# skygazer42/realtime-video-analytics-32streams

Measured on AMD Instinct MI355X. Metric: aggregate detected FPS across streams + p99 per-frame latency, 32x1080p30, higher is better.
Workload: dtype f16

## Files before the change

include/rva.h:

```cpp
#ifndef RVA_H
#define RVA_H

#include <stdint.h>

#ifdef __cplusplus
extern "C" {
#endif

#define RVA_ABI_VERSION 1

enum rva_status {
    RVA_OK = 0,
    RVA_ERR_ARG = 1,
    RVA_ERR_HIP = 2,
    RVA_ERR_CAPACITY = 3,
    RVA_ERR_UNAVAILABLE = 4
};

enum rva_dtype { RVA_F16 = 0, RVA_F32 = 1, RVA_F64 = 2  };

typedef struct rva_ctx rva_ctx;
typedef struct rva_tracker rva_tracker;
typedef void *rva_stream_t;

// ... 113 lines not shown
int rva_tracker_set_next_id(rva_tracker *trk, int64_t next_id, rva_stream_t stream);

int rva_conv_cout_pad(int Cout);
int rva_conv_num_variants(void);
const char *rva_conv_variant_name(int variant);
int rva_conv2d_nhwc_f16(rva_ctx *ctx, const void *in, int ldi, const void *weights, const float *bias,
                        void *out, int ldo, const void *residual, int ldr, int batch, int H, int W, int Cin,
                        int Cout, int ksize, int stride, int act, rva_stream_t stream);
int rva_conv2d_nhwc_f16_v(rva_ctx *ctx, const void *in, int ldi, const void *weights, const float *bias,
                          void *out, int ldo, const void *residual, int ldr, int batch, int H, int W, int Cin,
                          int Cout, int ksize, int stride, int act, int variant, rva_stream_t stream);
int rva_conv2d_nhwc_f16_rows(rva_ctx *ctx, const void *in, int ldi, const void *weights, const float *bias,
                             void *out, int ldo, const void *residual, int ldr, int batch, int H, int W, int Cin,
                             int Cout, int ksize, int stride, int act, int variant, int y0, int y1, rva_stream_t stream);
int rva_conv_rows_through(int k, int stride, int H_in, int lo, int hi, int32_t *out_lo, int32_t *out_hi);
int rva_conv1x1_upcat_f16(rva_ctx *ctx, const void *low, int ld_low, int c_low, const void *skip, int ld_skip,
                          int c_skip, const void *weights, const float *bias, void *out, int ldo, int batch,
                          int H, int W, int Cout, int act, int variant, rva_stream_t stream);
int rva_conv1x1_head_f16(rva_ctx *ctx, const void *in, int ldi, const void *weights, const float *bias, int batch,
                         int H, int W, int Cin, int Cout, int mode, void *out, int nc, int anchors_total,
                         int anchor_offset, float stride_px, int variant, rva_stream_t stream);
int rva_conv1x1_head_box32_f16(rva_ctx *ctx, const void *in, int ldi, const void *weights, const float *bias, int batch,
                               int H, int W, int Cin, void *out, float *boxes32, int nc, int anchors_total, int anchor_offset,
                               float stride_px, int variant, rva_stream_t stream);
int rva_stem_conv_f16(rva_ctx *ctx, const void *in_planar, const void *weights, const float *bias,
                      void *out, int ldo, int batch, int H, int W, int Cout, rva_stream_t stream);

int rva_c2f_pair32_f16(rva_ctx *ctx, const void *in, int ldi, const void *w1, const float *b1, const void *w2, const float *b2, void *out,
                       int ldo, int batch, int H, int W, rva_stream_t stream);

// ... 255 lines not shown
```

realtime_video_analytics_32streams_amd/_native.py:

```python
from __future__ import annotations

import ctypes as C
import os
import shutil
import subprocess
from pathlib import Path
from typing import Optional

PKG = Path(__file__).resolve().parent
ROOT = PKG.parent
CSRC = PKG / "csrc"
LIB_PATH = Path(os.environ["RVA_LIB_PATH"]) if os.environ.get("RVA_LIB_PATH") else PKG / "librva.so"
SOURCES = ["rva_ctx.hip", "rva_preprocess.hip", "rva_postprocess.hip", "rva_tracker.hip", "rva_conv.hip", "rva_conv_f32.hip", "rva_plan.hip", "rva_clip.hip",
           "rva_clip3d.hip", "rva_clip3d_f16.hip", "rva_clip_f16.hip", "rva_resnet.hip", "rva_resnet_f16.hip", "rva_gates.hip", "rva_decode.hip", "rva_preview.hip", "rva_jpeg.hip"]
HIPCC_FLAGS = ["--offload-arch=gfx950", "-O3", "-fPIC", "-shared", "-std=c++17", "-ffp-contract=off",
               "-Wall", "-Wno-unused-function"]

RVA_OK, RVA_ERR_ARG, RVA_ERR_HIP, RVA_ERR_CAPACITY, RVA_ERR_UNAVAILABLE = range(5)
RVA_F16, RVA_F32, RVA_F64 = 0, 1, 2
NORM_IMAGENET_F32, NORM_VIDEO_F32, NORM_IMAGENET_F64 = 0, 1, 2
LAYOUT_NCHW, LAYOUT_CNHW = 0, 1
RVA_MAX_BATCH = 64
RVA_CODEC_H264, RVA_CODEC_HEVC = 0, 1

# ... 50 lines not shown
    _fields_ = [("y", C.c_void_p), ("uv", C.c_void_p), ("out_bgr", C.c_void_p)] + [
        (n, C.c_int32) for n in ("pitch", "src_w", "src_h", "ratio", "dst_w", "dst_h", "rect_first", "n_rects", "glyph_first", "n_glyphs")]


RVA_PLAN_NO_STEM2 = 1
RVA_PLAN_NO_CIN_PAD = 2
RVA_PLAN_NO_PAIR32 = 4
RVA_PLAN_F32 = 8
RVA_PLAN_BOX_F32 = 16


def _stale() -> bool:
    if not LIB_PATH.exists():
        return True
    t = LIB_PATH.stat().st_mtime
    deps = [CSRC / s for s in SOURCES] + [CSRC / "rva_internal.h", CSRC / "rva_plan_topo.h", CSRC / "rva_mfma_f32.h", CSRC / "rva_mfma_f16.h", ROOT / "include" / "rva.h"]
    return any(d.exists() and d.stat().st_mtime > t for d in deps)


def build(force: bool = False, verbose: bool = False) -> Path:
    if not force and not _stale():
        return LIB_PATH
    hipcc = shutil.which("hipcc") or "/opt/rocm/bin/hipcc"
    if not Path(hipcc).exists():
        if LIB_PATH.exists():
            return LIB_PATH
        raise RuntimeError("hipcc not found and librva.so is not built")
    cmd = [hipcc, *HIPCC_FLAGS, f"-I{ROOT / 'include'}", "-o", str(LIB_PATH), *[str(CSRC / s) for s in SOURCES], "-ldl"]
    if verbose:
        print(" ".join(cmd))
    subprocess.check_call(cmd, cwd=str(CSRC))
# ... 73 lines not shown
        "rva_decoder_release": (C.c_int, [_P, C.c_int]),
        "rva_motion_nv12_batch": (C.c_int, [_P, pp, pp, i32p, pp, pp, C.c_int, C.c_int, C.c_int, _P, _P]),
        "rva_motion_nv12_masked_batch": (C.c_int, [_P, pp, pp, i32p, pp, pp, pp, C.c_int, C.c_int, C.c_int, _P, _P]),
        "rva_motion_bgr_batch": (C.c_int, [_P, pp, i32p, pp, pp, C.c_int, C.c_int, C.c_int, _P, _P]),
        "rva_preprocess_nv12_masked_batch": (C.c_int, [_P, pp, pp, i32p, pp, C.c_int, C.c_int, C.c_int, _P, C.c_int, C.c_int,
                                                       C.c_int, C.POINTER(Letterbox), _P]),
        "rva_resize_nv12_to_bgr_batch": (C.c_int, [_P, pp, pp, i32p, pp, C.c_int, C.c_int, C.c_int, _P, C.c_int, C.c_int, _P]),
        "rva_tracker_set_box_scale": (C.c_int, [_P, f64p]),
        "rva_conv_cout_pad": (C.c_int, [C.c_int]),
        "rva_conv_num_variants": (C.c_int, []),
        "rva_conv_variant_name": (C.c_char_p, [C.c_int]),
        "rva_conv2d_nhwc_f16": (C.c_int, [_P, _P, C.c_int, _P, _P, _P, C.c_int, _P, C.c_int] + [C.c_int] * 8 + [_P]),
        "rva_conv2d_nhwc_f16_v": (C.c_int, [_P, _P, C.c_int, _P, _P, _P, C.c_int, _P, C.c_int] + [C.c_int] * 9 + [_P]),
        "rva_conv2d_nhwc_f16_rows": (C.c_int, [_P, _P, C.c_int, _P, _P, _P, C.c_int, _P, C.c_int] + [C.c_int] * 11 + [_P]),
        "rva_conv_rows_through": (C.c_int, [C.c_int] * 5 + [i32p, i32p]),
        "rva_stem2_f16_rows": (C.c_int, [_P, _P, _P, _P, _P, _P, _P, C.c_int, C.c_int, C.c_int, C.c_int, C.c_int, C.c_int, _P]),
        "rva_stem_conv_f16": (C.c_int, [_P, _P, _P, _P, _P, C.c_int, C.c_int, C.c_int, C.c_int, C.c_int, _P]),
        "rva_stem2_f16": (C.c_int, [_P, _P, _P, _P, _P, _P, _P, C.c_int, C.c_int, C.c_int, C.c_int, _P]),
        "rva_c2f_pair32_f16": (C.c_int, [_P, _P, C.c_int, _P, _P, _P, _P, _P, C.c_int, C.c_int, C.c_int, C.c_int, _P]),
        "rva_conv1x1_head_f16": (C.c_int, [_P, _P, C.c_int, _P, _P, C.c_int, C.c_int, C.c_int, C.c_int, C.c_int, C.c_int, _P, C.c_int,
                                           C.c_int, C.c_int, C.c_float, C.c_int, _P]),
        "rva_conv1x1_head_box32_f16": (C.c_int, [_P, _P, C.c_int, _P, _P, C.c_int, C.c_int, C.c_int, C.c_int, _P, _P, C.c_int,
                                                 C.c_int, C.c_int, C.c_float, C.c_int, _P]),
        "rva_yolo_head_box32_f16": (C.c_int, [_P, _P, C.c_int, _P, C.c_int, _P, _P, C.c_int, C.c_int, C.c_int, C.c_int, C.c_int,
                                              C.c_int, C.c_float, _P]),
        "rva_yolo_head3_box32_f16": (C.c_int, [_P, pp, i32p, pp, i32p, _P, _P, C.c_int, i32p, i32p, C.c_int, C.c_int,
                                               C.POINTER(C.c_float), _P]),
        "rva_conv1x1_upcat_f16": (C.c_int, [_P, _P, C.c_int, C.c_int, _P, C.c_int, C.c_int, _P, _P, _P, C.c_int, C.c_int, C.c_int,
                                            C.c_int, C.c_int, C.c_int, C.c_int, _P]),
        "rva_yolo_head3_f16": (C.c_int, [_P, pp, i32p, pp, i32p, _P, C.c_int, i32p, i32p, C.c_int, C.c_int, C.POINTER(C.c_float), _P]),
# ... 88 lines not shown
    "rva_tracker_set_gates", "rva_tracker_snapshot_status", "rva_tracker_new_counts",
    "rva_tracker_assign_ids", "rva_tracker_read", "rva_tracker_read_all", "rva_tracker_snapshot_async",
    "rva_tracker_snapshot_fetch", "rva_tracker_state",
    "rva_tracker_set_next_id", "rva_preview_nv12", "rva_decode_available", "rva_decoder_create", "rva_decoder_destroy", "rva_decoder_feed",
    "rva_decoder_next_frame", "rva_decoder_release", "rva_motion_nv12_batch", "rva_motion_nv12_masked_batch", "rva_motion_bgr_batch",
    "rva_preprocess_nv12_masked_batch", "rva_resize_nv12_to_bgr_batch", "rva_tracker_set_box_scale", "rva_conv_cout_pad", "rva_conv_num_variants", "rva_conv_variant_name", "rva_conv2d_nhwc_f16", "rva_conv2d_nhwc_f16_v", "rva_stem_conv_f16", "rva_stem2_f16", "rva_c2f_pair32_f16",
    "rva_conv1x1_head_f16", "rva_conv1x1_upcat_f16", "rva_sppf_pool3_nhwc_f16", "rva_maxpool5_nhwc_f16", "rva_upsample2x_nhwc_f16", "rva_yolo_head_f16", "rva_yolo_head3_f16",
    "rva_conv_f32_num_variants", "rva_conv2d_nhwc_f32_v", "rva_stem_conv_f32", "rva_maxpool5_nhwc_f32", "rva_upsample2x_nhwc_f32",
    "rva_yolo_head_f32",
    "rva_postprocess_boxes_batch", "rva_conv1x1_head_box32_f16", "rva_yolo_head_box32_f16", "rva_yolo_head3_box32_f16",
    "rva_yolov8_plan_output_layout",
    "rva_yolov8_plan_create", "rva_yolov8_plan_destroy", "rva_yolov8_plan_info", "rva_yolov8_plan_run", "rva_yolov8_plan_run_lanes",
    "rva_yolov8_plan_run_range", "rva_yolov8_plan_tunable_desc", "rva_yolov8_plan_launch_tunable", "rva_yolov8_plan_set_variant",
    "rva_yolov8_plan_get_variant", "rva_yolov8_plan_set_static_rows", "rva_yolov8_plan_step_rows", "rva_yolov8_plan_run_n",
    "rva_yolov8_plan_run_lanes_n", "rva_yolov8_plan_run_range_n", "rva_yolov8_plan_primed_images", "rva_conv2d_nhwc_f16_rows",
    "rva_stem2_f16_rows", "rva_conv_rows_through", "rva_cnnlstm_plan_create", "rva_cnnlstm_plan_destroy", "rva_cnnlstm_plan_info", "rva_cnnlstm_plan_run",
    "rva_cnnlstm_plan_run_post", "rva_cnnlstm_plan_stage", "rva_cnnlstm_f16_plan_create", "rva_cnnlstm_f16_plan_destroy", "rva_cnnlstm_f16_plan_info",
    "rva_cnnlstm_f16_plan_run", "rva_cnnlstm_f16_plan_run_post", "rva_cnnlstm_f16_plan_stage", "rva_cnn3d_plan_create", "rva_cnn3d_plan_destroy", "rva_cnn3d_plan_info", "rva_cnn3d_plan_run",
    "rva_cnn3d_plan_run_post", "rva_cnn3d_plan_stage", "rva_cnn3d_f16_plan_create", "rva_cnn3d_f16_plan_destroy", "rva_cnn3d_f16_plan_info",
    "rva_cnn3d_f16_plan_run", "rva_cnn3d_f16_plan_run_post", "rva_cnn3d_f16_plan_stage", "rva_resnet_plan_create", "rva_resnet_plan_destroy", "rva_resnet_plan_info",
    "rva_resnet_plan_run", "rva_resnet_plan_run_post", "rva_resnet_plan_stage", "rva_resnet_f16_plan_create", "rva_resnet_f16_plan_destroy",
    "rva_resnet_f16_plan_info", "rva_resnet_f16_plan_run", "rva_resnet_f16_plan_run_post", "rva_resnet_f16_plan_stage", "rva_jpeg_max_bytes", "rva_jpeg_encode_bgr", "rva_jpeg_status",
    "rva_jpeg_batch_create", "rva_jpeg_batch_destroy", "rva_jpeg_batch_encode", "rva_preview_nv12_batch",
]


class Context:

    def __init__(self, device: int = 0):
        L = lib()
        h = _P()
# ... 42 lines not shown
```

realtime_video_analytics_32streams_amd/csrc/rva_conv.hip:

```cpp
#include <hip/hip_fp16.h>

#include <cstdlib>

#include "rva_internal.h"

namespace {

typedef _Float16 h8 __attribute__((ext_vector_type(8)));
typedef float f4 __attribute__((ext_vector_type(4)));
typedef unsigned int u4 __attribute__((ext_vector_type(4)));

struct ConvArgs {
    const __half *in; int ldi;
    const __half *w;
    const float *bias;
    __half *out; int ldo;
    union {
        const __half *res;
        float *hbox;
    };
    int ldr;
    int CoutPad;
    __half *hout; int hmode, hnc, hA, ha0, hW, hHW; float hstride;
    const __half *in2; int ldi2, c_split;
// ... 1083 lines not shown
{
    static_assert(WGM * WGN == 8, "eight waves");
    static_assert(NSLOT == 2 || NSLOT == 3, "ring depth");
    constexpr int TM = BM / WGM, TN = BN / WGN, FM = TM / 16, FN = TN / 16;
    constexpr int APIECES = (BM + 2 + 15) / 16;
    constexpr int WPIECES = 3 * BN / 16;
    constexpr int PIECES = APIECES + WPIECES;
    constexpr int SLOTH = PIECES * 512;
    constexpr int NP = (PIECES + 7) / 8;
    extern __shared__ __attribute__((aligned(16))) unsigned char smem[];
    __half *ring = (__half *)smem;

    const int tid = threadIdx.x, lane = tid & 63;
    const int wv = __builtin_amdgcn_readfirstlane(tid >> 6);
    const int wm = wv % WGM, wn = wv / WGM;
    const int n_tile = (blockIdx.x >> 3) % a.n_tiles, m_tile = ((blockIdx.x >> 3) / a.n_tiles) * 8 + (blockIdx.x & 7);
    if (m_tile >= a.m_tiles) return;
    const int P0 = m_tile * BM, n0 = n_tile * BN;
    const int HW = a.H * a.W;
    const int cpt = a.Cin >> 5;
    const int nsteps = 3 * cpt;
    const int wrow = 9 * a.Cin;

    const int lrow = lane >> 2, lp = lane & 3;
    const int my_pieces = (PIECES - wv + 7) / 8;
    unsigned poff0[NP], poff1[NP], poff2[NP];
#pragma unroll
    for (int k = 0; k < NP; ++k) {
        const int idx = wv + 8 * k;
        if (idx < APIECES) {
            const int r = idx * 16 + lrow;
            const unsigned c = (unsigned)(((lp - 2 * (r >> 2)) & 3) * 16);
// ... 213 lines not shown
    int H, W, Cin, Cout, CoutPad, act, n_tiles, M, m_tiles, apieces, map_off;
};

template <int BM, int BN, int WGM, int WGN, bool NOSEL = false, bool PADO = false>
__global__ void __launch_bounds__(512) __attribute__((amdgpu_waves_per_eu(BN <= 64 && BM <= 320 ? 4 : 2))) k_conv3_run(RunArgs a)
{
    static_assert(WGM * WGN == 8, "eight waves");
    constexpr int TM = BM / WGM, TN = BN / WGN, FM = TM / 16, FN = TN / 16;
    constexpr int WPIECES = 3 * BN / 16;
    constexpr int NPW = (WPIECES + 7) / 8;
    constexpr int MAXA = 5;
    extern __shared__ __attribute__((aligned(16))) unsigned char smem[];
    const int tid = threadIdx.x, lane = tid & 63;
    const int wv = __builtin_amdgcn_readfirstlane(tid >> 6);
    const int wm = wv % WGM, wn = wv / WGM;
    const int n_tile = (blockIdx.x >> 3) % a.n_tiles, m_tile = ((blockIdx.x >> 3) / a.n_tiles) * 8 + (blockIdx.x & 7);
    if (m_tile >= a.m_tiles) return;
    const int P0 = m_tile * BM, n0 = n_tile * BN;
    const int HW = a.H * a.W;
    const int cpt = a.Cin >> 5;
    const int nsteps = 3 * cpt;
    const int wrow = 9 * a.Cin;
    const int apieces = a.apieces;
    __half *act0 = (__half *)smem;
    __half *wt0 = act0 + (size_t)2 * apieces * 512;
    const unsigned lds_act = lds_addr(act0), lds_w = lds_addr(wt0);

    const int lrow = lane >> 2, lp = lane & 3;
    unsigned aoff[MAXA], woff[NPW];
    const int Wp = PADO ? a.W + 1 : a.W, HWp = (a.H + 1) * Wp;
    const float inv_wp = 1.0f / (float)Wp, inv_hwp = 1.0f / (float)HWp;
    unsigned long long amask[PADO ? MAXA : 1];
// ... 211 lines not shown
    return hipGetLastError();
}

template <int BM, int BN, int WGM, int WGN>
__global__ void __launch_bounds__(512) __attribute__((amdgpu_waves_per_eu(BM <= 128 && BN <= 64 ? 4 : 2))) k_conv3_s2run(RunArgs a)
{
    static_assert(WGM * WGN == 8, "eight waves");
    constexpr int TM = BM / WGM, TN = BN / WGN, FM = TM / 16, FN = TN / 16;
    constexpr int WPIECES = 3 * BN / 16, NPW = (WPIECES + 7) / 8;
    constexpr int BMO = (BM + 1 + 15) / 16 * 16;
    constexpr int AP = (BMO + BM) / 16, MAXA = (AP + 7) / 8;
    extern __shared__ __attribute__((aligned(16))) unsigned char smem[];
    const int tid = threadIdx.x, lane = tid & 63;
    const int wv = __builtin_amdgcn_readfirstlane(tid >> 6);
    const int wm = wv % WGM, wn = wv / WGM;
    const int n_tile = (blockIdx.x >> 3) % a.n_tiles, m_tile = ((blockIdx.x >> 3) / a.n_tiles) * 8 + (blockIdx.x & 7);
    if (m_tile >= a.m_tiles) return;
    const int P0 = m_tile * BM, n0 = n_tile * BN;
    const int Ho = a.H >> 1, Wo = a.W >> 1, Wp = Wo + 1, HWp = Ho * Wp;
    const int cpt = a.Cin >> 5, nsteps = 3 * cpt, wrow = 9 * a.Cin;
    __half *act0 = (__half *)smem;
    __half *wt0 = act0 + (size_t)3 * AP * 512;
    const unsigned lds_act = lds_addr(act0), lds_w = lds_addr(wt0);
    const int lrow = lane >> 2, lp = lane & 3;
    const float inv_wp = 1.0f / (float)Wp, inv_hwp = 1.0f / (float)HWp;
    const int batch = a.M / (Ho * Wo);
    unsigned aoff[MAXA], woff[NPW];
    unsigned long long am1[MAXA], am0[MAXA];
#pragma unroll
    for (int k = 0; k < MAXA; ++k) {
        const int r = (wv + 8 * k) * 16 + lrow;
        const bool odd = r < BMO;
// ... 157 lines not shown
}

template <int BM, int BN, int WGM, int WGN>
__global__ void __launch_bounds__(512) __attribute__((amdgpu_waves_per_eu(2))) k_conv3_chunk(RunArgs a)
{
    static_assert(WGM * WGN == 8, "eight waves");
    constexpr int TM = BM / WGM, TN = BN / WGN, FM = TM / 16, FN = TN / 16;
    static_assert(TM % 16 == 0 && TN % 16 == 0, "whole fragments per wave");
    constexpr int WPIECES = 9 * BN / 16;
    constexpr int NPW = (WPIECES + 7) / 8;
    constexpr int MAXA = 5;
    extern __shared__ __attribute__((aligned(16))) unsigned char smem[];
    const int tid = threadIdx.x, lane = tid & 63;
    const int wv = __builtin_amdgcn_readfirstlane(tid >> 6);
    const int wm = wv % WGM, wn = wv / WGM;
    const int n_tile = (blockIdx.x >> 3) % a.n_tiles, m_tile = ((blockIdx.x >> 3) / a.n_tiles) * 8 + (blockIdx.x & 7);
    if (m_tile >= a.m_tiles) return;
    const int P0 = m_tile * BM, n0 = n_tile * BN;
    const int HW = a.H * a.W;
    const int cpt = a.Cin >> 5;
    const int wrow = 9 * a.Cin;
    const int apieces = a.apieces;
    __half *act0 = (__half *)smem;
    __half *wt0 = act0 + (size_t)2 * apieces * 512;
    const unsigned lds_act = lds_addr(act0), lds_w = lds_addr(wt0);

    const int lrow = lane >> 2, lp = lane & 3;
    unsigned aoff[MAXA], woff[NPW];
#pragma unroll
    for (int k = 0; k < MAXA; ++k) {
        const int r = (wv + 8 * k) * 16 + lrow;
        const int q = min(max(P0 - a.W - 1 + r, 0), a.M - 1);
// ... 159 lines not shown
    static_assert(SUB == 1 || NSLOT == 2, "several K-steps per barrier: two-slot ring");
    static_assert(!UP || (KS == 1 && BK == 64), "the upsample + concat source form exists for 1x1 convolutions");
    constexpr int TM = BM / WGM, TN = BN / WGN, FM = TM / 16, FN = TN / 16;
    constexpr int RPP = 512 / BK;
    constexpr int LPR = BK / 8;
    constexpr int APIECES = BM / RPP, WPIECES = BN / RPP;
    constexpr int NA = (APIECES + 7) / 8, NW = (WPIECES + 7) / 8;
    constexpr int SLOTH = (BM + BN) * BK;
    constexpr int TAPS = KS * KS, PAD = KS / 2;
    extern __shared__ __attribute__((aligned(16))) unsigned char smem[];
    __half *ring = (__half *)smem;

    const int tid = threadIdx.x, lane = tid & 63;
    const int wv = __builtin_amdgcn_readfirstlane(tid >> 6);
    const int wm = wv % WGM, wn = wv / WGM;
    const int n_tile = (blockIdx.x >> 3) % a.n_tiles, m_tile = ((blockIdx.x >> 3) / a.n_tiles) * 8 + (blockIdx.x & 7);
    if (m_tile >= a.m_tiles) return;
    const int P0 = m_tile * BM, n0 = n_tile * BN;
    const int HoWo = a.wrows * a.Wo;
    const int cpt = a.Cin / BK;
    const int nsteps = TAPS * cpt;
    const int wrow = TAPS * a.Cin;

    const int lrow = lane / LPR, lp = lane % LPR;
    const int c8 = (BK == 64 ? (lp ^ lrow) : ((lp - 2 * (lrow >> 2)) & 3)) * 8;
    unsigned actr[NA], actr2[UP ? NA : 1];
    int avm[NA];
    const float inv_howo = 1.0f / (float)HoWo, inv_wo = 1.0f / (float)a.Wo;
#pragma unroll
    for (int k = 0; k < NA; ++k) {
        const int m = P0 + (wv + 8 * k) * RPP + lrow;
        actr[k] = (unsigned)(c8 * 2);
// ... 278 lines not shown
    constexpr int PROWS = STRIDE == 2 ? PH * 2 * CW : PH * CW;
    constexpr int RPP = 512 / CIN, LPR = CIN / 8;
    constexpr int PPIECES = (PROWS + RPP - 1) / RPP;
    constexpr int WPIECES = 9 * CO / RPP;
    constexpr int FN = CO / 16, KCH = CIN / 32;
    constexpr int SROW = CO + 8;
    static_assert(TH * TW * SROW * 2 <= PPIECES * 1024, "the output stage reuses a patch buffer");
    extern __shared__ __attribute__((aligned(16))) unsigned char smem[];
    __half *wl = (__half *)smem;
    __half *patch0 = wl + WPIECES * 512;
    const int tid = threadIdx.x, lane = tid & 63;
    const int wv = __builtin_amdgcn_readfirstlane(tid >> 6);
    const int lrow = lane / LPR, lp = lane % LPR;
    const int tiles_img = a.tiles_x * a.tiles_y;
    const int n0 = (int)(blockIdx.x % a.n_tiles) * CO;
    const int bid = blockIdx.x / a.n_tiles, nblk = gridDim.x / a.n_tiles;
    auto src_c8 = [&](int row) { return (CIN == 64 ? (lp ^ (row & 7)) : ((lp - 2 * (row >> 2)) & 3)) * 8; };
    auto lds_off = [&](int row, int c) { return CIN == 64 ? row * 64 + ((c ^ (row & 7)) << 3) : swz32(row, c); };

    float4 bvs[FN];
#pragma unroll
    for (int i = 0; i < FN; ++i) bvs[i] = *reinterpret_cast<const float4 *>(a.bias + min(n0 + 16 * i + (lane >> 4) * 4, a.CoutPad - 4));

#pragma unroll
    for (int k = 0; k < (WPIECES + NWV - 1) / NWV; ++k) {
        const int idx = wv + NWV * k;
        if (idx < WPIECES) {
            const int row = idx * RPP + lrow;
            const int tap = row / CO, co = min(n0 + row - tap * CO, a.CoutPad - 1);
            const __half *src = a.w + (size_t)(co * 9 + tap) * CIN + src_c8(row);
            __builtin_amdgcn_global_load_lds((glb_vptr)src, (lds_vptr)(wl + idx * 512), 16, 0, 0);
// ... 24 lines not shown
                const int q = ok ? (img + iy) * a.W + ix : 0;
                const __half *src = a.in + (size_t)q * a.ldi + pc8[k];
                __builtin_amdgcn_global_load_lds((glb_vptr)src, (lds_vptr)(dst + idx * 512), 16, 0, 0);
            }
        }
    };

    const h8 hz = {0, 0, 0, 0, 0, 0, 0, 0};
#ifdef RVA_ROW_STAMPS
    const int st_stride = gridDim.x / 8;
    const bool st_on = tid == 0 && st_stride > 0 && blockIdx.x % st_stride == 0 && blockIdx.x / st_stride < 8;
    const int st_slot = st_on ? blockIdx.x / st_stride : 0;
    int st_n = 0;
#endif
    int pb = 0;
    if (NBUF == 2 && bid < a.total) issue_patch(bid, 0);
    for (int t = bid; t < a.total; t += nblk) {
        STAMP(0);
        if (NBUF == 1) issue_patch(t, 0);
        wait_vm<0>();
        STAMP(1);
        __builtin_amdgcn_s_barrier();
        STAMP(2);
        if (NBUF == 2 && t + nblk < a.total) issue_patch(t + nblk, pb ^ 1);
        STAMP(3);
        const __half *patch = patch0 + (size_t)pb * PPIECES * 512;
        __half *stage = patch0 + (size_t)pb * PPIECES * 512;
        const int b = t / tiles_img, r2 = t - b * tiles_img, ty = r2 / a.tiles_x, tx = r2 - ty * a.tiles_x;
        int vm[FMW];
#pragma unroll
        for (int j = 0; j < FMW; ++j) {
            const int oy = a.y0 + ty * TH + wv * RPW + (j >> 1);
            const int ox = tx * TW + 16 * (j & 1) + (lane & 15);
            int m = 0;
            if (oy < a.y1 && ox < a.Wo) {
#pragma unroll
                for (int tp = 0; tp < 9; ++tp)
                    if ((unsigned)(STRIDE * oy - 1 + tp / 3) < (unsigned)a.H && (unsigned)(STRIDE * ox - 1 + tp % 3) < (unsigned)a.W) m |= 1 << tp;
            }
// ... 137 lines not shown
    }
    int ppy[NIP], ppx[NIP], pc8[NIP];
#pragma unroll
    for (int k = 0; k < NIP; ++k) {
        const int row = (wv + NWV * k) * 16 + lrow;
        ppy[k] = row < (TH + 4) * PITCH ? row / PITCH : 1 << 20;
        ppx[k] = row % PITCH;
        pc8[k] = ((lp - 2 * (row >> 2)) & 3) * 8;
    }
    int mmy[NMF], mmx[NMF];
#pragma unroll
    for (int k = 0; k < NMF; ++k) {
        const int row = (wv + NWV * k) * 16 + n;
        mmy[k] = row / PITCH; mmx[k] = row % PITCH;
    }
    for (int t = blockIdx.x; t < a.total; t += gridDim.x) {
        const int b = t / tiles_img, r2 = t - b * tiles_img, ty = r2 / a.tiles_x, tx = r2 - ty * a.tiles_x;
        const int y0 = ty * TH, x0 = tx * TW;
#pragma unroll
        for (int k = 0; k < NIP; ++k) {
            const int idx = wv + NWV * k;
            if (idx < PR_IPIECES) {
                const int iy = y0 - 2 + ppy[k], ix = x0 - 2 + ppx[k];
                const bool ok = (unsigned)iy < (unsigned)a.H && (unsigned)ix < (unsigned)a.W;
                const __half *src = ok ? a.in + ((size_t)(b * a.H + iy) * a.W + ix) * a.ldi + pc8[k] : reinterpret_cast<const __half *>(g_zero_line);
                __builtin_amdgcn_global_load_lds((glb_vptr)src, (lds_vptr)(inp + idx * 512), 16, 0, 0);
            }
        }
        wait_vm<0>();
        __syncthreads();
        f4 acc1[NMF][2];
// ... 139 lines not shown
            if (idx < PPIECES) {
                const bool ok = (unsigned)(iy_base + (pgeo[k] >> 8)) < (unsigned)a.H && (unsigned)(ix_base + (pgeo[k] & 255)) < (unsigned)a.W;
                lds_dma16(ok ? poff[k] : centre, base, lds_patch + (unsigned)idx * 1024u);
            }
        }
    };
    const h8 hz = {0, 0, 0, 0, 0, 0, 0, 0};
    int boff[RPW + 2][3];
#pragma unroll
    for (int r = 0; r < RPW + 2; ++r)
#pragma unroll
        for (int dx = 0; dx < 3; ++dx) boff[r][dx] = lds_off((ws * RPW + r) * CW + dx + n, q);
    const int aoff = lds_off(n, q);
    float *bias_l = reinterpret_cast<float *>(patch0 + (size_t)2 * PPIECES * 512);
    if (tid < CO) bias_l[tid] = a.bias[min(tid, a.CoutPad - 1)];
    const int nblk_tiles = (int)blockIdx.x < a.total ? (a.total - (int)blockIdx.x + (int)gridDim.x - 1) / (int)gridDim.x : 0;
    const int nmine = (nblk_tiles - set + 1) / 2;
    const int niter = (nblk_tiles + 1) / 2;
#ifdef RVA_ROW_STAMPS
    const int st_stride = gridDim.x / 4;
    const bool st_on = (tid == 0 || tid == SW * 64) && st_stride > 0 && blockIdx.x % st_stride == 0 && blockIdx.x / st_stride < 4;
    const int st_slot = st_on ? (blockIdx.x / st_stride) * 2 + (tid >= SW * 64 ? 1 : 0) : 0;
    int st_n = 0;
#endif
    if (nmine > 0) issue_patch(blockIdx.x + set * gridDim.x);
    wait_vm<0>();
    __builtin_amdgcn_s_barrier();
    if (set == 1) __builtin_amdgcn_s_barrier();
    for (int it = 0; it < niter; ++it) {
        const bool live = it < nmine;
        const int t = blockIdx.x + (2 * it + set) * gridDim.x;
        const int b = t / tiles_img, r2 = t - b * tiles_img, ty = r2 / a.tiles_x, tx = r2 - ty * a.tiles_x;
        STAMP(0);
        f4 acc[FN][FMW];
        if (live) {
            int vm[FMW];
#pragma unroll
            for (int j = 0; j < FMW; ++j) {
                const int oy = a.y0 + ty * TH + ws * RPW + (j >> 1), ox = tx * TW + 16 * (j & 1) + n;
                int m = 0;
                if (oy < a.y1 && ox < a.Wo) {
                    const int hv = (ox >= 1 ? 1 : 0) | 2 | (ox <= a.W - 2 ? 4 : 0);
                    m = (oy >= 1 ? hv : 0) | (hv << 3) | (oy <= a.H - 2 ? hv << 6 : 0);
                }
                vm[j] = m;
            }
// ... 38 lines not shown
                P2_PAIR(0); P2_PAIR(2); P2_PAIR(4); P2_PAIR(6); P2_PAIR(8); P2_PAIR(10); P2_PAIR(12); P2_PAIR(14);
                P2_LOAD(bfb, afb, 17); P2_MFMA(bfa, afa, 16); P2_MFMA(bfb, afb, 17);
            } else {
                P2_ONE(0); P2_ONE(1); P2_ONE(2); P2_ONE(3); P2_ONE(4); P2_ONE(5); P2_ONE(6); P2_ONE(7); P2_ONE(8);
                P2_ONE(9); P2_ONE(10); P2_ONE(11); P2_ONE(12); P2_ONE(13); P2_ONE(14); P2_ONE(15); P2_ONE(16); P2_ONE(17);
                (void)bfb; (void)afb;
            }
#undef P2_ONE
#undef P2_PAIR
#undef P2_LOAD
#undef P2_MFMA
        }
        STAMP(1);
        __builtin_amdgcn_s_barrier();
        STAMP(2);
        if (it + 1 < nmine) issue_patch(t + 2 * gridDim.x);
        STAMP(3);
        if (live) {
            const int qh = q & 1, qc = q >> 1;
            const int ox = tx * TW + 16 * qh + n;
#pragma unroll
            for (int r = 0; r < RPW; ++r) {
                const int oy = a.y0 + ty * TH + ws * RPW + r;
                const bool pv = oy < a.y1 && ox < a.Wo;
                const size_t m = (size_t)(b * a.Ho + oy) * a.Wo + ox;
#pragma unroll
                for (int i = 0; i < FN; ++i) {
                    const float4 bv = *reinterpret_cast<const float4 *>(bias_l + 16 * i + q * 4);
                    uint32_t w2[2][2];
#pragma unroll
                    for (int h = 0; h < 2; ++h) {
// ... 67 lines not shown
{
    constexpr int TH = S2_TH, TW = S2_TW, CW = TW + 1, PROWS = S2_PROWS, WPIECES = 9 * 64 / 16;
    constexpr int IR = S2_IR, IC = S2_IC;
    constexpr int NCH = 3 * IR * (IC / 8), NPV = (NCH + 511) / 512;
    constexpr int SPX = (2 * TH + 1) * (2 * TW + 1), NFR = (SPX + 15) / 16;
    constexpr int SROW = S2_SROW, FN = 4;
    extern __shared__ __attribute__((aligned(16))) unsigned char smem[];
    __half *wl = (__half *)smem;
    __half *patch0 = wl + WPIECES * 512;
    __half *inp0 = patch0 + 2 * (PROWS + 1) * 32;
    __half *stage0 = inp0 + 2 * 3 * IR * IC;
    const int tid = threadIdx.x, lane = tid & 63;
    const int wv = __builtin_amdgcn_readfirstlane(tid >> 6);
    const int n = lane & 15, q = lane >> 4;
    const int tiles_img = a.tiles_x * a.tiles_y;
    const int nk = ((int)a.total - (int)blockIdx.x + (int)gridDim.x - 1) / (int)gridDim.x;

    {
        const int lrow = lane >> 2, lp = lane & 3;
#pragma unroll
        for (int k = 0; k < (WPIECES + 15) / 16; ++k) {
            const int idx = wv + 16 * k;
            if (idx < WPIECES) {
                const int row = idx * 16 + lrow;
                const int tap = row >> 6, co = row & 63;
                const __half *src = a.w2 + (size_t)(co * 9 + tap) * 32 + ((lp - 2 * (row >> 2)) & 3) * 8;
                __builtin_amdgcn_global_load_lds((glb_vptr)src, (lds_vptr)(wl + idx * 512), 16, 0, 0);
            }
        }
    }
#ifdef RVA_ROW_STAMPS
// ... 48 lines not shown
            }
        };
        constexpr int FPW = (NFR + 7) / 8, UNR = FPW;
        static_assert(FPW % UNR == 0, "fragments per wave");
        int frd[FPW], fpp[FPW], fw[FPW];
#pragma unroll
        for (int e = 0; e < FPW; ++e) {
            const int f = wv + 8 * e;
            const int p = min(16 * f + n, SPX - 1);
            const int py = p / (2 * TW + 1), px = p - py * (2 * TW + 1);
            const int prow = (py * 2 + (px & 1)) * CW + (px >> 1);
            frd[e] = (2 * py) * IC + 2 * px + 4;
            fpp[e] = (py << 8) | px;
            fw[e] = 16 * f + n < SPX ? swz32(prow, q >> 1) + 4 * (q & 1) : PROWS * 32 + 4 * (q & 1);
        }
        if (nk > 0) { prefetch(blockIdx.x); stage_input(0); }
        __syncthreads();
        for (int k = 0; k <= nk; ++k) {
            STAMP(0);
            if (k < nk) {
                const int t = blockIdx.x + k * gridDim.x;
                const int b = t / tiles_img, r2 = t - b * tiles_img, ty = r2 / a.tiles_x, tx = r2 - ty * a.tiles_x;
                (void)b;
                if (k + 1 < nk) prefetch(t + gridDim.x);
                const __half *inp = inp0 + (size_t)(k & 1) * 3 * IR * IC;
                __half *patch = patch0 + (size_t)(k & 1) * (PROWS + 1) * 32;
                const int sy0 = 2 * (a.y0 + ty * TH) - 1, sx0 = 2 * tx * TW - 1;
                const int pyb = -sy0, pxb = -sx0;
                const int pye = a.H1 - sy0, pxe = a.W1 - sx0;
#pragma unroll
                for (int g = 0; g < FPW / UNR; ++g) {
                    h8 bf1[UNR], bf2[UNR];
#pragma unroll
                    for (int u = 0; u < UNR; ++u) {
                        const __half *base = inp + frd[g * UNR + u];
                        const uint32_t *d0 = reinterpret_cast<const uint32_t *>(base + ro0), *d1 = reinterpret_cast<const uint32_t *>(base + ro1);
                        const uint32_t *d8 = reinterpret_cast<const uint32_t *>(base + ro8);
                        uint32_t b1w[4] = {d0[0], d0[1], d1[0], d1[1]};
                        uint32_t b2w[4] = {d8[0], d8[1], 0u, 0u};
// ... 30 lines not shown
            STAMP(2);
            __syncthreads();
            STAMP(3);
        }
    } else {
        const int wb = wv - 8, orow = wb >> 1, ohalf = wb & 1;
        float4 bvs[FN];
#pragma unroll
        for (int i = 0; i < FN; ++i) bvs[i] = *reinterpret_cast<const float4 *>(a.b2 + 16 * i + q * 4);
        wait_vm<0>();
        __syncthreads();
        __half *stage = stage0 + (size_t)wb * 16 * SROW;
        for (int k = 0; k <= nk; ++k) {
            STAMP(0);
            if (k > 0) {
                const int t = blockIdx.x + (k - 1) * gridDim.x;
                const int b = t / tiles_img, r2 = t - b * tiles_img, ty = r2 / a.tiles_x, tx = r2 - ty * a.tiles_x;
                const __half *patch = patch0 + (size_t)((k - 1) & 1) * (PROWS + 1) * 32;
                f4 acc[FN];
#pragma unroll
                for (int i = 0; i < FN; ++i) acc[i] = f4{bvs[i].x, bvs[i].y, bvs[i].z, bvs[i].w};
#pragma unroll
                for (int tp = 0; tp < 9; ++tp) {
                    const int dy = tp / 3, dx = tp % 3;
                    const int rb = ((2 * orow + dy) * 2 + (dx & 1)) * CW + (dx >> 1) + 16 * ohalf + n;
                    const h8 bf = *reinterpret_cast<const h8 *>(patch + swz32(rb, q));
#pragma unroll
                    for (int i = 0; i < FN; ++i) {
                        const h8 af = *reinterpret_cast<const h8 *>(wl + swz32(tp * 64 + 16 * i + n, q));
                        acc[i] = __builtin_amdgcn_mfma_f32_16x16x32_f16(af, bf, acc[i], 0, 0, 0);
                    }
// ... 497 lines not shown
    if (!boxes32 || (uintptr_t)boxes32 % 4 || anchor_offset < 0 || anchor_offset + H * W > anchors_total)
        return rva_fail(ctx, RVA_ERR_ARG, "rva_conv1x1_head_box32_f16: boxes32 must be a float tensor [batch, 4, anchors_total] and the level must lie inside it");
    return conv1x1_head(ctx, in, ldi, weights, bias, batch, H, W, Cin, 64, 1, out, boxes32, nc, anchors_total, anchor_offset, stride_px, variant, stream_);
}

int rva_conv_cout_pad(int Cout) { return rva_ceil_div(Cout, 64) * 64; }

int rva_conv_num_variants(void) { return kConvVariantsMax; }

const char *rva_conv_variant_name(int variant)
{
    const ConvVariant *row = find_variant(variant);
    return row ? row->name : nullptr;
}

int rva_stem_conv_f16(rva_ctx *ctx, const void *in_planar, const void *weights, const float *bias, void *out, int ldo,
                      int batch, int H, int W, int Cout, rva_stream_t stream_)
{
    if (!ctx || !in_planar || !weights || !bias || !out || Cout % 8 || Cout > 64 || ldo % 8)
        return rva_fail(ctx, RVA_ERR_ARG, "rva_stem_conv_f16: bad argument");
    StemArgs a{(const __half *)in_planar, nullptr, bias, (__half *)out, batch, H, W, (H - 1) / 2 + 1, (W - 1) / 2 + 1, Cout, ldo};
#ifdef RVA_ROW_STAMPS
    { const char *e = getenv("RVA_STEM_DBG"); a.dbg = e ? atoi(e) : 0; }
#endif
    const int total_tiles = rva_ceil_div(a.Wo, 32) * rva_ceil_div(a.Ho, 8) * batch;
    int grid = 256 * 4;
    if (grid > total_tiles) grid = total_tiles;
    if (W % 8 || ((uintptr_t)in_planar & 15)) return rva_fail(ctx, RVA_ERR_ARG, "rva_stem_conv_f16: W %% 8 == 0 and a 16-byte aligned input are required");
    k_stem<<<grid, 256, (size_t)(3 * 17 * 88 * 2) + (size_t)(256 * (Cout + 8 > LDSROW ? Cout + 8 : LDSROW) + 64 * LDSROW) * 2, (hipStream_t)stream_>>>(a, (const __half *)weights, bias);
    RVA_HIP(ctx, hipGetLastError());
// ... 163 lines not shown
```

Measured before the change: 23760.

## Band tile-to-block mapping across conv kernels for locality

Result: no change. 23880 (median of 3 runs) (+0.5%).

```diff
diff --git a/include/rva.h b/include/rva.h
--- a/include/rva.h
+++ b/include/rva.h
@@ -151,6 +151,20 @@
                              void *out, int ldo, const void *residual, int ldr, int batch, int H, int W, int Cin,
                              int Cout, int ksize, int stride, int act, int variant, int y0, int y1, rva_stream_t stream);
 int rva_conv_rows_through(int k, int stride, int H_in, int lo, int hi, int32_t *out_lo, int32_t *out_hi);
+enum rva_tile_family {
+    RVA_TILE_FAMILY_BIG = 0,
+    RVA_TILE_FAMILY_RUN = 1,
+    RVA_TILE_FAMILY_CHUNK = 2,
+    RVA_TILE_FAMILY_S2RUN = 3,
+    RVA_TILE_FAMILY_GBIG = 4,
+    RVA_TILE_FAMILY_PATCH = 5,
+    RVA_TILE_FAMILY_PATCH2 = 6,
+    RVA_TILE_FAMILY_STEM2 = 7,
+    RVA_TILE_FAMILY_PAIR32 = 8,
+    RVA_TILE_FAMILY_COUNT = 9
+};
+int rva_conv_tile_of_block(int family, int bid, int grid, int m_tiles, int n_tiles, int32_t *m_tile, int32_t *n_tile);
+int rva_conv_tile_family_banded(int family);
 int rva_conv1x1_upcat_f16(rva_ctx *ctx, const void *low, int ld_low, int c_low, const void *skip, int ld_skip,
                           int c_skip, const void *weights, const float *bias, void *out, int ldo, int batch,
                           int H, int W, int Cout, int act, int variant, rva_stream_t stream);
diff --git a/realtime_video_analytics_32streams_amd/_native.py b/realtime_video_analytics_32streams_amd/_native.py
--- a/realtime_video_analytics_32streams_amd/_native.py
+++ b/realtime_video_analytics_32streams_amd/_native.py
@@ -88,7 +88,7 @@
     if not LIB_PATH.exists():
         return True
     t = LIB_PATH.stat().st_mtime
-    deps = [CSRC / s for s in SOURCES] + [CSRC / "rva_internal.h", CSRC / "rva_plan_topo.h", CSRC / "rva_mfma_f32.h", CSRC / "rva_mfma_f16.h", ROOT / "include" / "rva.h"]
+    deps = [CSRC / s for s in SOURCES] + [CSRC / "rva_internal.h", CSRC / "rva_plan_topo.h", CSRC / "rva_mfma_f32.h", CSRC / "rva_mfma_f16.h", CSRC / "rva_tile_order.h", ROOT / "include" / "rva.h"]
     return any(d.exists() and d.stat().st_mtime > t for d in deps)
 
 
@@ -192,6 +192,8 @@
         "rva_conv2d_nhwc_f16_v": (C.c_int, [_P, _P, C.c_int, _P, _P, _P, C.c_int, _P, C.c_int] + [C.c_int] * 9 + [_P]),
         "rva_conv2d_nhwc_f16_rows": (C.c_int, [_P, _P, C.c_int, _P, _P, _P, C.c_int, _P, C.c_int] + [C.c_int] * 11 + [_P]),
         "rva_conv_rows_through": (C.c_int, [C.c_int] * 5 + [i32p, i32p]),
+        "rva_conv_tile_of_block": (C.c_int, [C.c_int] * 5 + [i32p, i32p]),
+        "rva_conv_tile_family_banded": (C.c_int, [C.c_int]),
         "rva_stem2_f16_rows": (C.c_int, [_P, _P, _P, _P, _P, _P, _P, C.c_int, C.c_int, C.c_int, C.c_int, C.c_int, C.c_int, _P]),
         "rva_stem_conv_f16": (C.c_int, [_P, _P, _P, _P, _P, C.c_int, C.c_int, C.c_int, C.c_int, C.c_int, _P]),
         "rva_stem2_f16": (C.c_int, [_P, _P, _P, _P, _P, _P, _P, C.c_int, C.c_int, C.c_int, C.c_int, _P]),
@@ -310,7 +312,7 @@
     "rva_yolov8_plan_run_range", "rva_yolov8_plan_tunable_desc", "rva_yolov8_plan_launch_tunable", "rva_yolov8_plan_set_variant",
     "rva_yolov8_plan_get_variant", "rva_yolov8_plan_set_static_rows", "rva_yolov8_plan_step_rows", "rva_yolov8_plan_run_n",
     "rva_yolov8_plan_run_lanes_n", "rva_yolov8_plan_run_range_n", "rva_yolov8_plan_primed_images", "rva_conv2d_nhwc_f16_rows",
-    "rva_stem2_f16_rows", "rva_conv_rows_through", "rva_cnnlstm_plan_create", "rva_cnnlstm_plan_destroy", "rva_cnnlstm_plan_info", "rva_cnnlstm_plan_run",
+    "rva_stem2_f16_rows", "rva_conv_rows_through", "rva_conv_tile_of_block", "rva_conv_tile_family_banded", "rva_cnnlstm_plan_create", "rva_cnnlstm_plan_destroy", "rva_cnnlstm_plan_info", "rva_cnnlstm_plan_run",
     "rva_cnnlstm_plan_run_post", "rva_cnnlstm_plan_stage", "rva_cnnlstm_f16_plan_create", "rva_cnnlstm_f16_plan_destroy", "rva_cnnlstm_f16_plan_info",
     "rva_cnnlstm_f16_plan_run", "rva_cnnlstm_f16_plan_run_post", "rva_cnnlstm_f16_plan_stage", "rva_cnn3d_plan_create", "rva_cnn3d_plan_destroy", "rva_cnn3d_plan_info", "rva_cnn3d_plan_run",
     "rva_cnn3d_plan_run_post", "rva_cnn3d_plan_stage", "rva_cnn3d_f16_plan_create", "rva_cnn3d_f16_plan_destroy", "rva_cnn3d_f16_plan_info",
diff --git a/realtime_video_analytics_32streams_amd/csrc/rva_conv.hip b/realtime_video_analytics_32streams_amd/csrc/rva_conv.hip
--- a/realtime_video_analytics_32streams_amd/csrc/rva_conv.hip
+++ b/realtime_video_analytics_32streams_amd/csrc/rva_conv.hip
@@ -3,6 +3,7 @@
 #include <cstdlib>
 
 #include "rva_internal.h"
+#include "rva_tile_order.h"
 
 namespace {
 
@@ -1121,8 +1122,8 @@
     const int tid = threadIdx.x, lane = tid & 63;
     const int wv = __builtin_amdgcn_readfirstlane(tid >> 6);
     const int wm = wv % WGM, wn = wv / WGM;
-    const int n_tile = (blockIdx.x >> 3) % a.n_tiles, m_tile = ((blockIdx.x >> 3) / a.n_tiles) * 8 + (blockIdx.x & 7);
-    if (m_tile >= a.m_tiles) return;
+    int m_tile, n_tile;
+    if (!rva_tile_of_block(rva_tiles_banded(RVA_TILES_BIG), blockIdx.x, a.m_tiles, a.n_tiles, m_tile, n_tile)) return;
     const int P0 = m_tile * BM, n0 = n_tile * BN;
     const int HW = a.H * a.W;
     const int cpt = a.Cin >> 5;
@@ -1366,8 +1367,8 @@
     const int tid = threadIdx.x, lane = tid & 63;
     const int wv = __builtin_amdgcn_readfirstlane(tid >> 6);
     const int wm = wv % WGM, wn = wv / WGM;
-    const int n_tile = (blockIdx.x >> 3) % a.n_tiles, m_tile = ((blockIdx.x >> 3) / a.n_tiles) * 8 + (blockIdx.x & 7);
-    if (m_tile >= a.m_tiles) return;
+    int m_tile, n_tile;
+    if (!rva_tile_of_block(rva_tiles_banded(RVA_TILES_RUN), blockIdx.x, a.m_tiles, a.n_tiles, m_tile, n_tile)) return;
     const int P0 = m_tile * BM, n0 = n_tile * BN;
     const int HW = a.H * a.W;
     const int cpt = a.Cin >> 5;
@@ -1609,8 +1610,8 @@
     const int tid = threadIdx.x, lane = tid & 63;
     const int wv = __builtin_amdgcn_readfirstlane(tid >> 6);
     const int wm = wv % WGM, wn = wv / WGM;
-    const int n_tile = (blockIdx.x >> 3) % a.n_tiles, m_tile = ((blockIdx.x >> 3) / a.n_tiles) * 8 + (blockIdx.x & 7);
-    if (m_tile >= a.m_tiles) return;
+    int m_tile, n_tile;
+    if (!rva_tile_of_block(rva_tiles_banded(RVA_TILES_S2RUN), blockIdx.x, a.m_tiles, a.n_tiles, m_tile, n_tile)) return;
     const int P0 = m_tile * BM, n0 = n_tile * BN;
     const int Ho = a.H >> 1, Wo = a.W >> 1, Wp = Wo + 1, HWp = Ho * Wp;
     const int cpt = a.Cin >> 5, nsteps = 3 * cpt, wrow = 9 * a.Cin;
@@ -1798,8 +1799,8 @@
     const int tid = threadIdx.x, lane = tid & 63;
     const int wv = __builtin_amdgcn_readfirstlane(tid >> 6);
     const int wm = wv % WGM, wn = wv / WGM;
-    const int n_tile = (blockIdx.x >> 3) % a.n_tiles, m_tile = ((blockIdx.x >> 3) / a.n_tiles) * 8 + (blockIdx.x & 7);
-    if (m_tile >= a.m_tiles) return;
+    int m_tile, n_tile;
+    if (!rva_tile_of_block(rva_tiles_banded(RVA_TILES_CHUNK), blockIdx.x, a.m_tiles, a.n_tiles, m_tile, n_tile)) return;
     const int P0 = m_tile * BM, n0 = n_tile * BN;
     const int HW = a.H * a.W;
     const int cpt = a.Cin >> 5;
@@ -1989,8 +1990,8 @@
     const int tid = threadIdx.x, lane = tid & 63;
     const int wv = __builtin_amdgcn_readfirstlane(tid >> 6);
     const int wm = wv % WGM, wn = wv / WGM;
-    const int n_tile = (blockIdx.x >> 3) % a.n_tiles, m_tile = ((blockIdx.x >> 3) / a.n_tiles) * 8 + (blockIdx.x & 7);
-    if (m_tile >= a.m_tiles) return;
+    int m_tile, n_tile;
+    if (!rva_tile_of_block(rva_tiles_banded(RVA_TILES_GBIG), blockIdx.x, a.m_tiles, a.n_tiles, m_tile, n_tile)) return;
     const int P0 = m_tile * BM, n0 = n_tile * BN;
     const int HoWo = a.wrows * a.Wo;
     const int cpt = a.Cin / BK;
@@ -2299,7 +2300,7 @@
     const int lrow = lane / LPR, lp = lane % LPR;
     const int tiles_img = a.tiles_x * a.tiles_y;
     const int n0 = (int)(blockIdx.x % a.n_tiles) * CO;
-    const int bid = blockIdx.x / a.n_tiles, nblk = gridDim.x / a.n_tiles;
+    const rva_walk wk = rva_tile_walk(rva_tiles_banded(RVA_TILES_PATCH), blockIdx.x / a.n_tiles, gridDim.x / a.n_tiles, a.total, rva_walk_groups(a.n_tiles));
     auto src_c8 = [&](int row) { return (CIN == 64 ? (lp ^ (row & 7)) : ((lp - 2 * (row >> 2)) & 3)) * 8; };
     auto lds_off = [&](int row, int c) { return CIN == 64 ? row * 64 + ((c ^ (row & 7)) << 3) : swz32(row, c); };
 
@@ -2354,15 +2355,15 @@
     int st_n = 0;
 #endif
     int pb = 0;
-    if (NBUF == 2 && bid < a.total) issue_patch(bid, 0);
-    for (int t = bid; t < a.total; t += nblk) {
+    if (NBUF == 2 && wk.count > 0) issue_patch(wk.first, 0);
+    for (int k = 0, t = wk.first; k < wk.count; ++k, t += wk.step) {
         STAMP(0);
         if (NBUF == 1) issue_patch(t, 0);
         wait_vm<0>();
         STAMP(1);
         __builtin_amdgcn_s_barrier();
         STAMP(2);
-        if (NBUF == 2 && t + nblk < a.total) issue_patch(t + nblk, pb ^ 1);
+        if (NBUF == 2 && k + 1 < wk.count) issue_patch(t + wk.step, pb ^ 1);
         STAMP(3);
         const __half *patch = patch0 + (size_t)pb * PPIECES * 512;
         __half *stage = patch0 + (size_t)pb * PPIECES * 512;
@@ -2530,7 +2531,8 @@
         const int row = (wv + NWV * k) * 16 + n;
         mmy[k] = row / PITCH; mmx[k] = row % PITCH;
     }
-    for (int t = blockIdx.x; t < a.total; t += gridDim.x) {
+    const rva_walk wk = rva_tile_walk(rva_tiles_banded(RVA_TILES_PAIR32), blockIdx.x, gridDim.x, a.total);
+    for (int it = 0, t = wk.first; it < wk.count; ++it, t += wk.step) {
         const int b = t / tiles_img, r2 = t - b * tiles_img, ty = r2 / a.tiles_x, tx = r2 - ty * a.tiles_x;
         const int y0 = ty * TH, x0 = tx * TW;
 #pragma unroll
@@ -2700,7 +2702,8 @@
     const int aoff = lds_off(n, q);
     float *bias_l = reinterpret_cast<float *>(patch0 + (size_t)2 * PPIECES * 512);
     if (tid < CO) bias_l[tid] = a.bias[min(tid, a.CoutPad - 1)];
-    const int nblk_tiles = (int)blockIdx.x < a.total ? (a.total - (int)blockIdx.x + (int)gridDim.x - 1) / (int)gridDim.x : 0;
+    const rva_walk wk = rva_tile_walk(rva_tiles_banded(RVA_TILES_PATCH2), blockIdx.x, gridDim.x, a.total);
+    const int nblk_tiles = wk.count;
     const int nmine = (nblk_tiles - set + 1) / 2;
     const int niter = (nblk_tiles + 1) / 2;
 #ifdef RVA_ROW_STAMPS
@@ -2709,13 +2712,13 @@
     const int st_slot = st_on ? (blockIdx.x / st_stride) * 2 + (tid >= SW * 64 ? 1 : 0) : 0;
     int st_n = 0;
 #endif
-    if (nmine > 0) issue_patch(blockIdx.x + set * gridDim.x);
+    if (nmine > 0) issue_patch(wk.first + set * wk.step);
     wait_vm<0>();
     __builtin_amdgcn_s_barrier();
     if (set == 1) __builtin_amdgcn_s_barrier();
     for (int it = 0; it < niter; ++it) {
         const bool live = it < nmine;
-        const int t = blockIdx.x + (2 * it + set) * gridDim.x;
+        const int t = wk.first + (2 * it + set) * wk.step;
         const int b = t / tiles_img, r2 = t - b * tiles_img, ty = r2 / a.tiles_x, tx = r2 - ty * a.tiles_x;
         STAMP(0);
         f4 acc[FN][FMW];
@@ -2784,7 +2787,7 @@
         STAMP(1);
         __builtin_amdgcn_s_barrier();
         STAMP(2);
-        if (it + 1 < nmine) issue_patch(t + 2 * gridDim.x);
+        if (it + 1 < nmine) issue_patch(t + 2 * wk.step);
         STAMP(3);
         if (live) {
             const int qh = q & 1, qc = q >> 1;
@@ -2882,7 +2885,8 @@
     const int wv = __builtin_amdgcn_readfirstlane(tid >> 6);
     const int n = lane & 15, q = lane >> 4;
     const int tiles_img = a.tiles_x * a.tiles_y;
-    const int nk = ((int)a.total - (int)blockIdx.x + (int)gridDim.x - 1) / (int)gridDim.x;
+    const rva_walk wk = rva_tile_walk(rva_tiles_banded(RVA_TILES_STEM2), blockIdx.x, gridDim.x, a.total);
+    const int nk = wk.count;
 
     {
         const int lrow = lane >> 2, lp = lane & 3;
@@ -2961,15 +2965,15 @@
             fpp[e] = (py << 8) | px;
             fw[e] = 16 * f + n < SPX ? swz32(prow, q >> 1) + 4 * (q & 1) : PROWS * 32 + 4 * (q & 1);
         }
-        if (nk > 0) { prefetch(blockIdx.x); stage_input(0); }
+        if (nk > 0) { prefetch(wk.first); stage_input(0); }
         __syncthreads();
         for (int k = 0; k <= nk; ++k) {
             STAMP(0);
             if (k < nk) {
-                const int t = blockIdx.x + k * gridDim.x;
+                const int t = wk.first + k * wk.step;
                 const int b = t / tiles_img, r2 = t - b * tiles_img, ty = r2 / a.tiles_x, tx = r2 - ty * a.tiles_x;
                 (void)b;
-                if (k + 1 < nk) prefetch(t + gridDim.x);
+                if (k + 1 < nk) prefetch(t + wk.step);
                 const __half *inp = inp0 + (size_t)(k & 1) * 3 * IR * IC;
                 __half *patch = patch0 + (size_t)(k & 1) * (PROWS + 1) * 32;
                 const int sy0 = 2 * (a.y0 + ty * TH) - 1, sx0 = 2 * tx * TW - 1;
@@ -3030,7 +3034,7 @@
         for (int k = 0; k <= nk; ++k) {
             STAMP(0);
             if (k > 0) {
-                const int t = blockIdx.x + (k - 1) * gridDim.x;
+                const int t = wk.first + (k - 1) * wk.step;
                 const int b = t / tiles_img, r2 = t - b * tiles_img, ty = r2 / a.tiles_x, tx = r2 - ty * a.tiles_x;
                 const __half *patch = patch0 + (size_t)((k - 1) & 1) * (PROWS + 1) * 32;
                 f4 acc[FN];
@@ -3558,6 +3562,31 @@
     return row ? row->name : nullptr;
 }
 
+static_assert(RVA_TILES_BIG == RVA_TILE_FAMILY_BIG && RVA_TILES_RUN == RVA_TILE_FAMILY_RUN && RVA_TILES_CHUNK == RVA_TILE_FAMILY_CHUNK &&
+              RVA_TILES_S2RUN == RVA_TILE_FAMILY_S2RUN && RVA_TILES_GBIG == RVA_TILE_FAMILY_GBIG && RVA_TILES_PATCH == RVA_TILE_FAMILY_PATCH &&
+              RVA_TILES_PATCH2 == RVA_TILE_FAMILY_PATCH2 && RVA_TILES_STEM2 == RVA_TILE_FAMILY_STEM2 && RVA_TILES_PAIR32 == RVA_TILE_FAMILY_PAIR32 &&
+              RVA_TILES_FAMILIES == RVA_TILE_FAMILY_COUNT, "rva_tile_order.h and enum rva_tile_family");
+
+int rva_conv_tile_of_block(int family, int bid, int grid, int m_tiles, int n_tiles, int32_t *m_tile, int32_t *n_tile)
+{
+    if (family < 0 || family >= RVA_TILES_FAMILIES || !m_tile || !n_tile || bid < 0 || grid <= 0 || m_tiles <= 0 || n_tiles <= 0) return RVA_ERR_ARG;
+    const bool banded = rva_tiles_banded(family);
+    int m = -1, n = -1;
+    if (family <= RVA_TILES_GBIG) {
+        if ((long long)grid != 8LL * rva_ceil_div(m_tiles, 8) * n_tiles || bid >= grid) return RVA_ERR_ARG;
+        if (!rva_tile_of_block(banded, bid, m_tiles, n_tiles, m, n)) m = n = -1;
+    } else {
+        if (grid % n_tiles || (family != RVA_TILES_PATCH && n_tiles != 1)) return RVA_ERR_ARG;
+        const int blk = bid % grid, k = bid / grid;
+        const rva_walk wk = rva_tile_walk(banded, blk / n_tiles, grid / n_tiles, m_tiles, rva_walk_groups(n_tiles));
+        if (k < wk.count) { m = wk.first + k * wk.step; n = blk % n_tiles; }
+    }
+    *m_tile = m; *n_tile = n;
+    return RVA_OK;
+}
+
+int rva_conv_tile_family_banded(int family) { return family < 0 || family >= RVA_TILES_FAMILIES ? -1 : rva_tiles_banded(family) ? 1 : 0; }
+
 int rva_stem_conv_f16(rva_ctx *ctx, const void *in_planar, const void *weights, const float *bias, void *out, int ldo,
                       int batch, int H, int W, int Cout, rva_stream_t stream_)
 {
diff --git a/realtime_video_analytics_32streams_amd/csrc/rva_tile_order.h b/realtime_video_analytics_32streams_amd/csrc/rva_tile_order.h
--- /dev/null
+++ b/realtime_video_analytics_32streams_amd/csrc/rva_tile_order.h
@@ -0,0 +1,65 @@
+#pragma once
+
+#define RVA_TILES_BIG 0
+#define RVA_TILES_RUN 1
+#define RVA_TILES_CHUNK 2
+#define RVA_TILES_S2RUN 3
+#define RVA_TILES_GBIG 4
+#define RVA_TILES_PATCH 5
+#define RVA_TILES_PATCH2 6
+#define RVA_TILES_STEM2 7
+#define RVA_TILES_PAIR32 8
+#define RVA_TILES_FAMILIES 9
+
+#ifndef RVA_TILE_ORDER_OLD_MASK
+#ifdef RVA_TILE_ORDER_OLD
+#define RVA_TILE_ORDER_OLD_MASK 0x1ff
+#else
+#define RVA_TILE_ORDER_OLD_MASK (1 << RVA_TILES_PATCH)
+#endif
+#endif
+
+#if defined(__HIPCC__) || defined(__CUDACC__)
+#define RVA_HD __host__ __device__
+#else
+#define RVA_HD
+#endif
+
+constexpr bool rva_tiles_banded(int family) { return !((RVA_TILE_ORDER_OLD_MASK >> family) & 1); }
+
+RVA_HD inline bool rva_tile_of_block(bool banded, int bid, int m_tiles, int n_tiles, int &m_tile, int &n_tile)
+{
+    const int x = bid & 7, slot = bid >> 3;
+    const int i = slot / n_tiles;
+    n_tile = slot - i * n_tiles;
+    if (!banded) {
+        m_tile = i * 8 + x;
+        return m_tile < m_tiles;
+    }
+    const int q = m_tiles >> 3, r = m_tiles & 7;
+    m_tile = x * q + (x < r ? x : r) + i;
+    return i < q + (x < r ? 1 : 0);
+}
+
+struct rva_walk { int first, step, count; };
+
+RVA_HD inline int rva_walk_groups(int n_tiles) { return n_tiles == 2 || n_tiles == 4 || n_tiles == 8 ? 8 / n_tiles : 8; }
+
+RVA_HD inline rva_walk rva_tile_walk(bool banded, int bid, int nblk, int total, int groups = 8)
+{
+    rva_walk w;
+    if (!banded) {
+        w.first = bid; w.step = nblk;
+        w.count = bid < total ? (total - bid + nblk - 1) / nblk : 0;
+        return w;
+    }
+    const int g = bid % groups, j = bid / groups;
+    const int q = nblk / groups, r = nblk % groups;
+    const int nb = q + (g < r ? 1 : 0);
+    const int before = g * q + (g < r ? g : r);
+    const int start = (int)((unsigned long long)total * (unsigned)before / (unsigned)nblk);
+    const int end = (int)((unsigned long long)total * (unsigned)(before + nb) / (unsigned)nblk);
+    w.first = start + j; w.step = nb;
+    w.count = j < end - start ? (end - start - j + nb - 1) / nb : 0;
+    return w;
+}
```
